# olsonanl/signature_kmers

Measured on AMD Instinct MI355X. Metric: k-mers/sec (extract+hash+count) at 1/2/4/8 GPUs; achieved HBM GB/s %, higher is better.
Workload: dtype u8

## Files before the change

### signature_kmers_amd/csrc/skm_build.hip

```cpp
#include <hip/hip_runtime.h>

#include <algorithm>
#include <type_traits>
#include <chrono>
#include <cmath>
#include <cstdio>
#include <cstdlib>
#include <cstring>
#include <deque>
#include <functional>
#include <memory>
#include <numeric>
#include <string>
#include <thread>
#include <vector>

#include "skm_common.h"
#include "skm_pool.h"
#include "skm_output.h"
#include "skm_util.h"

#if defined(SKM_WITH_RCCL)
#include <rccl/rccl.h>
#endif
// ... 2098 lines not shown
        }
#pragma unroll
        for (int t = 0; t < SC_POS; ++t)
            rk[t] = agg_rank(L.cnt, sb[t], base + threadIdx.x + (uint64_t)t * EX_THREADS < end);
        __syncthreads();
        const uint32_t tot = stage_reserve(L, nsub, cur1, b0 << sub_bits);
#pragma unroll
        for (int t = 0; t < SC_POS; ++t) {
            const uint64_t j = base + threadIdx.x + (uint64_t)t * EX_THREADS;
            if (j < end) {
                const uint32_t slot = L.off[sb[t]] + rk[t];
                L.hi[slot] = eh[t];
                L.lo[slot] = el[t];
                L.dst[slot] = (uint8_t)sb[t];
            }
        }
        __syncthreads();
        for (uint32_t j = threadIdx.x; j < tot; j += blockDim.x) {
            const uint32_t d = L.dst[j];
            const uint64_t o = L.base[d] + (j - L.off[d]);
            out_hi[o] = L.hi[j];
            out_lo[o] = L.lo[j];
        }
        __syncthreads();
    }
}

__global__ void k_colsum(const uint32_t* __restrict__ hist, uint32_t nwg, uint32_t NB, uint32_t* __restrict__ partial) {
    uint32_t b = blockIdx.x * blockDim.x + threadIdx.x;
    uint32_t rb = blockIdx.y;
    if (b >= NB) return;
    uint32_t w0 = rb * SCAN_ROWS, w1 = min(nwg, w0 + SCAN_ROWS);
    uint32_t s = 0;
    for (uint32_t w = w0; w < w1; ++w) s += hist[(uint64_t)w * NB + b];
    partial[(uint64_t)rb * NB + b] = s;
}

__global__ void k_bstart(const uint32_t* __restrict__ partial, uint32_t nrb, uint32_t NB, int b1_bits,
                         uint32_t* __restrict__ rbbase, uint32_t* __restrict__ bstart, uint64_t* __restrict__ owner_start,
                         uint32_t nowners) {
    __shared__ uint32_t s_wave[34];
    __shared__ unsigned long long s_tot[64];
    const uint32_t per = (NB + blockDim.x - 1) / blockDim.x;
    const uint32_t b0 = threadIdx.x * per;
    uint32_t local = 0;
    for (uint32_t b = b0; b < min(NB, b0 + per); ++b) {
        uint32_t acc = 0;
        for (uint32_t rb = 0; rb < nrb; ++rb) {
            uint32_t v = partial[(uint64_t)rb * NB + b];
            rbbase[(uint64_t)rb * NB + b] = acc;
            acc += v;
        }
        bstart[b] = acc;
        local += acc;
    }
    uint32_t total;
    uint32_t ex = wg_exclusive_scan(local, s_wave, total);
    uint32_t run = ex;
    for (uint32_t b = b0; b < min(NB, b0 + per); ++b) {
        uint32_t t = bstart[b];
        bstart[b] = run;
        run += t;
    }
    __syncthreads();
    if (threadIdx.x < nowners) {
        uint32_t ob = threadIdx.x << b1_bits;
        s_tot[threadIdx.x] = bstart[ob];
    }
    if (threadIdx.x == 0) s_tot[nowners] = total;
    __syncthreads();
    if (threadIdx.x <= nowners) owner_start[threadIdx.x] = s_tot[threadIdx.x];
    for (uint32_t b = b0; b < min(NB, b0 + per); ++b) {
        uint32_t o = b >> b1_bits;
        uint32_t rel = bstart[b] - (uint32_t)s_tot[o];
        for (uint32_t rb = 0; rb < nrb; ++rb) rbbase[(uint64_t)rb * NB + b] += rel;
    }
    __syncthreads();
    for (uint32_t b = b0; b < min(NB, b0 + per); ++b) bstart[b] -= (uint32_t)s_tot[b >> b1_bits];
    if (threadIdx.x == 0) bstart[NB] = 0;
}

__global__ void k_coloffs(const uint32_t* __restrict__ hist, const uint32_t* __restrict__ rbbase, uint32_t nwg, uint32_t NB,
                          uint32_t* __restrict__ offs) {
    uint32_t b = blockIdx.x * blockDim.x + threadIdx.x;
    uint32_t rb = blockIdx.y;
    if (b >= NB) return;
    uint32_t w0 = rb * SCAN_ROWS, w1 = min(nwg, w0 + SCAN_ROWS);
    uint32_t run = rbbase[(uint64_t)rb * NB + b];
    for (uint32_t w = w0; w < w1; ++w) {
        uint64_t idx = (uint64_t)w * NB + b;
        uint32_t v = hist[idx];
        offs[idx] = run;
        run += v;
    }
}

struct BucketArgs {
    uint64_t* recs_hi;
    const uint64_t* recs_lo;
    uint64_t* tmp_hi;
    uint64_t* tmp_lo;
    const uint64_t* bstart;
    const uint64_t* seg_start;
    const uint32_t* seg_len;
    uint32_t nsrc;
    uint32_t* sub_tab;
    unsigned long long* kept_ctr;

    uint32_t nbuckets;
    uint32_t bucket_base;
    int rem_bits;
    const uint32_t* glen;
    uint8_t* flags;
    unsigned long long* ctr;
    uint64_t* out_keys;
    skm_stored_kmer_data* out_data;
    Job* jobs;
    uint32_t* lens;
    OvfEntry* ovf;
    uint32_t ovf_cap;
    unsigned long long* stamps;
    uint64_t* big_desc;
    uint32_t big_cap;
    unsigned long long* big_ctr;
    int prio;
    int pshift;
    int flag_check;
    const uint32_t* skip;
    uint32_t sub_target;
    int diag;
    const uint32_t* order;
    int part_class;
};

#define SKM_STAMP(i)                                                          \
    do {                                                                      \
        if (A.stamps && threadIdx.x == 0) {                                   \
            const uint64_t _t = __builtin_amdgcn_s_memtime();                 \
            atomicAdd(&A.stamps[(i)], (unsigned long long)(_t - *L.tlast));   \
            *L.tlast = _t;                                                    \
        }                                                                     \
    } while (0)

constexpr uint32_t JOB_KEPT = 0x8000u;
constexpr uint32_t JOB_COUNT_MASK = 0x0FFFu;

struct SubLds {
    uint64_t* hi;
    uint64_t* lo;
    uint32_t* tab;
    uint16_t* slot;
    uint16_t* rank;
    uint16_t* goff;
    uint16_t* glist;
    uint16_t* order;
    uint16_t* big;
    uint32_t* wave;
    uint32_t* nbig;
    uint64_t* tlast;
    uint32_t* ccnt;
    uint32_t* lens32;
    uint64_t lens_sel;
};

__device__ __forceinline__ uint64_t kept_hi(uint64_t h43, uint32_t avg) { return (1ull << 63) | (h43 << 16) | avg; }
__device__ __forceinline__ uint64_t kept_lo(uint32_t f, uint32_t mean, uint32_t med, uint32_t var) {
    return (uint64_t)f | ((uint64_t)mean << 16) | ((uint64_t)med << 32) | ((uint64_t)var << 48);
}

__device__ __forceinline__ void write_kept(const BucketArgs& A, uint64_t o, uint64_t H, uint64_t L) {
    A.out_keys[o] = (H >> 16) & KEY_MASK;
    skm_stored_kmer_data d;
    d.avg_from_end = (uint16_t)(H & 0xFFFFu);
    d.function_index = (uint16_t)(L & 0xFFFFu);
    d.mean = (uint16_t)(L >> 16);
    d.median = (uint16_t)(L >> 32);
    d.var = (uint16_t)(L >> 48);
    A.out_data[o] = d;
}



__device__ __forceinline__ uint64_t shfl_xor_u64(uint64_t v, int m) {
    return ((uint64_t)(uint32_t)__shfl_xor((int)(uint32_t)(v >> 32), m, 64) << 32) |
           (uint32_t)__shfl_xor((int)(uint32_t)v, m, 64);
}


__device__ __forceinline__ void bm_combine(uint32_t& cand, uint32_t& cc) {
#pragma unroll
    for (int d = 1; d < 64; d <<= 1) {
        const uint32_t oc = xs(cand, d), on = xs(cc, d);
        if (oc == cand) {
            cc += on;
        } else if (cc >= on) {
            cc -= on;
        } else {
            cand = oc;
            cc = on - cc;
        }
    }
    cand = (uint32_t)__shfl((int)cand, 0, 64);
}


template <int S>
__device__ __forceinline__ uint64_t seg_bitonic64(uint64_t key, uint32_t& pay, uint32_t m) {
#pragma unroll
    for (int k = 2; k <= S; k <<= 1) {
#pragma unroll
        for (int j = k >> 1; j > 0; j >>= 1) {
            const uint64_t ok = xs64(key, j);
            const uint32_t op = xs(pay, j);
            const bool take_min = ((m & (uint32_t)j) == 0) == ((m & (uint32_t)k) == 0);
            if (take_min ? (ok < key) : (ok > key)) {
                key = ok;
                pay = op;
            }
        }
    }
    return key;
}

template <int S>
__device__ __forceinline__ uint32_t seg_bitonic32(uint32_t key, uint32_t m) {
#pragma unroll
    for (int k = 2; k <= S; k <<= 1) {
#pragma unroll
        for (int j = k >> 1; j > 0; j >>= 1) {
            const uint32_t ok = xs(key, j);
            const bool take_min = ((m & (uint32_t)j) == 0) == ((m & (uint32_t)k) == 0);
            key = take_min ? min(key, ok) : max(key, ok);
        }
    }
    return key;
}

template <int S>
__device__ __forceinline__ uint32_t seg_reduce_max(uint32_t x) {
#pragma unroll
    for (int d = 1; d < S; d <<= 1) x = max(x, xs(x, d));
    return x;
}

template <int S>
__device__ __forceinline__ uint32_t seg_reduce_sum(uint32_t x) {
#pragma unroll
    for (int d = 1; d < S; d <<= 1) x += xs(x, d);
    return x;
}

template <int S>
__device__ __forceinline__ void seg_groups(const SubLds& L, uint32_t q0, uint32_t qend, uint32_t G, uint32_t M,
                                           const BucketArgs& A, uint64_t hprefix, uint32_t* jobinfo,
                                           uint32_t* fmean) {
    const uint32_t lane = threadIdx.x & 63u;
    const uint32_t m = lane & (uint32_t)(S - 1);
    const uint32_t sbase = lane - m;
    const uint32_t q = q0 + lane / (uint32_t)S;
    const bool gv = q < qend;
    uint32_t rep = 0, a = 0, c = 0;
    if (gv) {
        const uint32_t g = L.big[q];
        rep = L.glist[g];
        a = L.goff[rep];
        c = (g + 1 < G ? L.goff[L.glist[g + 1]] : M) - a;
    }
    const bool real = gv && m < c;
    uint64_t key = ~0ull;
    uint32_t pay = 0;
    if (real) {
        const uint32_t j = L.order[a + m];
        const uint64_t hj = L.hi[j], lj = L.lo[j];
        key = ((hj & 0xFFFFull) << 48) | (lj >> 16);
        pay = (uint32_t)(hj >> 47);
    }
    key = seg_bitonic64<S>(key, pay, m);
    const uint32_t f = (uint32_t)(key >> 48);
    const uint32_t fprev = (uint32_t)__shfl_up((int)f, 1, 64);
    const bool head = !real || m == 0 || f != fprev;
    const uint64_t H = __ballot(head);
    const uint64_t above = lane == 63 ? 0ull : (H & ~((2ull << lane) - 1ull));
    const uint32_t nh = above ? (uint32_t)__ffsll((long long)above) - 1u : 64u;
    const uint32_t rlen = min(nh, sbase + c) - lane;
    const uint32_t v = (real && head) ? ((rlen << 16) | (0xFFFFu - f)) : 0u;
    const uint32_t best = seg_reduce_max<S>(v);
    const uint32_t cbest = best >> 16, bf = 0xFFFFu - (best & 0xFFFFu);
    const bool kept = gv && !((float)cbest < float(c) * 0.8f);
    const bool inrun = real && f == bf;
    const uint32_t len16 = pay >> 1;
    const uint32_t sum = seg_reduce_sum<S>(inrun ? len16 : 0u);
    const uint32_t i = (uint32_t)(key & ((1u << ELEM_I_BITS) - 1));
    const uint32_t off = real ? ((len16 - i) & 0xFFFFu) : 0x10000u;
    const uint32_t osort = seg_bitonic32<S>(off, m);
    const uint32_t avg = (uint32_t)__shfl((int)osort, (int)(sbase + (c >> 1)), 64);
    const uint64_t R = __ballot(inrun);
    const uint64_t segmask = (S == 64) ? ~0ull : (((1ull << S) - 1ull) << sbase);
    const uint64_t Rs = R & segmask;
    const uint32_t rs = Rs ? (uint32_t)__ffsll((long long)Rs) - 1u : sbase;
    const uint32_t s = (uint32_t)(key >> ELEM_I_BITS) & ((1u << ELEM_S_BITS) - 1u);
    const uint32_t fl = (A.flag_check && real && A.flags) ? A.flags[s] : 0u;
    const uint32_t len = (pay & 1u) ? A.glen[s] : len16;
    if (kept && real && fl == 0 && A.flags) mark_seq(A.flags, s);
    const uint32_t x0 = (uint32_t)__shfl((int)len, (int)(rs + cbest - 1), 64);
    const uint32_t x1 = (uint32_t)__shfl((int)len, (int)rs, 64);
    if (kept && inrun && cbest >= 3) L.lens32[2 * a + (rs + cbest - 1 - lane)] = len;
    if (kept && m == 0) {
        GRes r;
        r.kept = true;
        r.best_f = bf;
        r.cbest = cbest;
        r.avg = avg;
        r.mean = d2u16((double)(uint16_t)sum / (double)cbest);
        stats_small(r, x0, cbest == 2 ? x1 : 0u, cbest);
        const uint64_t h43 = key_h43(hprefix, (L.hi[rep] >> 16) & REM_MASK, A.rem_bits, A.pshift);
        L.hi[rep] = kept_hi(h43, r.avg);
        if (cbest >= 3) {
            jobinfo[rep] = (a << 16) | JOB_KEPT | cbest;
            fmean[rep] = bf | ((uint32_t)r.mean << 16);
        } else {
            jobinfo[rep] = JOB_KEPT;
            L.lo[rep] = kept_lo(bf, r.mean, r.median, r.var);
        }
    }
}

constexpr uint32_t LPER = CAP / BPK_THREADS;

__device__ __forceinline__ void load_batch(const uint64_t* __restrict__ src_hi, const uint64_t* __restrict__ src_lo,
                                           uint32_t n, uint64_t (&eh)[LPER], uint64_t (&el)[LPER]) {
#pragma unroll
    for (uint32_t u = 0; u < LPER; ++u) {
        const uint32_t j = threadIdx.x + u * BPK_THREADS;
        if (j < n) {
            eh[u] = __builtin_nontemporal_load(src_hi + j);
            el[u] = __builtin_nontemporal_load(src_lo + j);
        }
    }
}

__device__ __forceinline__ uint32_t process_sub(const uint64_t* __restrict__ src_hi, const uint64_t* __restrict__ src_lo,
                                            uint32_t n, const BucketArgs& A, uint64_t hprefix, const SubLds& L) {
    const uint32_t tid = threadIdx.x, nt = blockDim.x;
    const uint32_t EMPTY = 0xFFFFFFFFu;
    uint64_t eh[LPER], el[LPER];
    load_batch(src_hi, src_lo, n, eh, el);
    for (uint32_t t = tid; t < (uint32_t)TAB; t += nt) L.tab[t] = EMPTY;
#pragma unroll
    for (uint32_t u = 0; u < LPER; ++u) {
        const uint32_t j = tid + u * BPK_THREADS;
        if (j < n) {
            L.hi[j] = eh[u];
            L.lo[j] = el[u];
        }
    }
    if (tid == 0) *L.nbig = 0;
    if (tid < 8) L.ccnt[tid] = 0;
    __syncthreads();
    SKM_STAMP(2);
    for (uint32_t j = tid; j < n; j += nt) {
        const uint32_t rem = (uint32_t)(L.hi[j] >> 16) & REM_MASK;
        uint32_t slot = (rem * 0x9E3779B1u) >> (32 - TAB_BITS);
        uint32_t rk = 0;
        while (true) {
            const uint32_t cur = atomicCAS(&L.tab[slot], EMPTY, (j << 16) | 1u);
            if (cur == EMPTY) break;
            if (((uint32_t)(L.hi[cur >> 16] >> 16) & REM_MASK) == rem) {
                rk = atomicAdd(&L.tab[slot], 1u) & 0xFFFFu;
                break;
            }
            slot = (slot + 1) & (TAB - 1);
        }
        L.slot[j] = (uint16_t)slot;
        L.rank[j] = (uint16_t)rk;
    }
    __syncthreads();
    SKM_STAMP(3);
    uint32_t M = 0, G = 0;
    {
        const uint32_t j0 = tid * LPER;
        uint32_t ev[LPER], loc = 0;
#pragma unroll
        for (uint32_t u = 0; u < LPER; ++u) {
            const uint32_t j = j0 + u;
            ev[u] = j < n ? L.tab[L.slot[j]] : 0u;
            const uint32_t cnt = ev[u] & 0xFFFFu;
            loc += (cnt > 1 && (ev[u] >> 16) == j) ? ((cnt << 13) | 1u) : 0u;
        }
        uint32_t tot;
        uint32_t v = wg_exclusive_scan1(loc, L.wave, tot);
        uint32_t ms[LPER];
#pragma unroll
        for (uint32_t u = 0; u < LPER; ++u) {
            const uint32_t j = j0 + u;
            const uint32_t cnt = ev[u] & 0xFFFFu;
            ms[u] = 0xFFFFFFFFu;
            if (j < n && cnt > 1 && (ev[u] >> 16) == j) {
                L.goff[j] = (uint16_t)(v >> 13);
                L.glist[v & 0x1FFFu] = (uint16_t)j;
                v += (cnt << 13) | 1u;
            } else if (j < n && cnt == 1) {
                const uint64_t H = L.hi[j], Lo = L.lo[j];
                ms[u] = (uint32_t)(Lo >> 36);
                L.hi[j] = kept_hi(key_h43(hprefix, (H >> 16) & REM_MASK, A.rem_bits, A.pshift), (uint32_t)(Lo & 0xFFFFu));
                L.lo[j] = kept_lo((uint32_t)(H & 0xFFFFu), d2u16((double)(uint16_t)(H >> 48) / 1.0), 0, 0);
                L.rank[j] = 0xFFFFu;
            }
        }
        if (A.flags) mark_seqs<LPER>(A.flags, A.flag_check, ms);
        M = tot >> 13;
        G = tot & 0x1FFFu;
    }
    __syncthreads();
    SKM_STAMP(4);
    for (uint32_t j = tid; j < n; j += nt) {
        const uint32_t e = L.tab[L.slot[j]];
        if ((e & 0xFFFFu) > 1) L.order[L.goff[e >> 16] + L.rank[j]] = (uint16_t)j;
    }
    uint32_t* ccnt = L.ccnt;
    auto cls_of = [](uint32_t c) -> uint32_t {
        return c > 64u ? 6u : 31u - (uint32_t)__clz(c - 1u) - 0u;
    };
    for (uint32_t g = tid; g < G; g += nt) {
        const uint32_t a = L.goff[L.glist[g]];
        const uint32_t c = g + 1 < G ? L.goff[L.glist[g + 1]] - a : M - a;
        atomicAdd(&ccnt[cls_of(c)], 1u);
    }
    __syncthreads();
    SKM_STAMP(5);
    uint32_t* jobinfo = L.tab;
    uint32_t* fmean = L.tab + CAP;
    for (uint32_t j = tid; j < n; j += nt) jobinfo[j] = L.rank[j] == 0xFFFFu ? JOB_KEPT : 0u;
    uint32_t* cstart = ccnt + 8;
    uint32_t* tstart = ccnt + 16;
    if (tid == 0) {
        uint32_t run = 0, acc = 0;
        for (int q = 0; q < 7; ++q) {
            const uint32_t t = ccnt[q];
            ccnt[q] = run;
            cstart[q] = run;
            tstart[q] = acc;
            const uint32_t per = q < 6 ? (64u >> (q + 1)) : 1u;
            acc += (t + per - 1) / per;
            run += t;
        }
        cstart[7] = run;
        tstart[7] = acc;
    }
    unsigned long long big_base = 0;
    if (tid == 0 && cstart[7] > cstart[6]) big_base = atomicAdd(A.big_ctr, (unsigned long long)(cstart[7] - cstart[6]));
    __syncthreads();
    for (uint32_t g = tid; g < G; g += nt) {
        const uint32_t a = L.goff[L.glist[g]];
        const uint32_t c = g + 1 < G ? L.goff[L.glist[g + 1]] - a : M - a;
        L.big[atomicAdd(&ccnt[cls_of(c)], 1u)] = (uint16_t)g;
    }
    if (tid == 0) *reinterpret_cast<unsigned long long*>(L.wave + 44) = big_base;
    __syncthreads();
    SKM_STAMP(6);
    {
        const uint32_t ntask = tstart[6];
        const uint32_t nbig = cstart[7] - cstart[6];
        const uint64_t bbase = *reinterpret_cast<const unsigned long long*>(L.wave + 44);
        const uint32_t wave = tid >> 6, nwaves = nt >> 6, lane = tid & 63u;
        uint64_t* slots = reinterpret_cast<uint64_t*>(L.lens32);
        uint64_t* slots_lo = const_cast<uint64_t*>(src_lo);
        (void)wave;
        (void)nwaves;
        for (;;) {
            uint32_t t = 0;
            if (lane == 0) t = atomicAdd(&ccnt[7], 1u);
            t = (uint32_t)__builtin_amdgcn_readfirstlane((int)t);
            if (t >= nbig + ntask) break;
            if (t < nbig) {
                const uint32_t g = L.big[cstart[6] + t];
                const uint32_t rep = L.glist[g];
                const uint32_t a = L.goff[rep];
                const uint32_t c = g + 1 < G ? L.goff[L.glist[g + 1]] - a : M - a;
                for (uint32_t u = lane; u < c; u += 64) {
                    const uint32_t j = L.order[a + u];
                    const uint64_t hj = L.hi[j], lj = L.lo[j];
                    slots[a + u] = ((hj & 0xFFFFull) << 48) | (lj >> 16);
                    slots_lo[a + u] = elem_len(hj, lj, A.glen);
                }
                const uint64_t q = bbase + t;
                if (lane == 0 && q < A.big_cap) {
                    A.big_desc[2 * q] = key_h43(hprefix, (L.hi[rep] >> 16) & REM_MASK, A.rem_bits, A.pshift) |
                                        ((uint64_t)c << KEY_BITS);
                    A.big_desc[2 * q + 1] = L.lens_sel + 2 * a;
                }
                continue;
            }
            const uint32_t ts = ntask - 1u - (t - nbig);
            uint32_t k = 0;
            while (k < 5 && ts >= tstart[k + 1]) ++k;
            const uint32_t per = 64u >> (k + 1);
            const uint32_t q0 = cstart[k] + (ts - tstart[k]) * per, qe = cstart[k + 1];
            switch (k) {
                case 0: seg_groups<2>(L, q0, qe, G, M, A, hprefix, jobinfo, fmean); break;
                case 1: seg_groups<4>(L, q0, qe, G, M, A, hprefix, jobinfo, fmean); break;
                case 2: seg_groups<8>(L, q0, qe, G, M, A, hprefix, jobinfo, fmean); break;
                case 3: seg_groups<16>(L, q0, qe, G, M, A, hprefix, jobinfo, fmean); break;
                case 4: seg_groups<32>(L, q0, qe, G, M, A, hprefix, jobinfo, fmean); break;
                default: seg_groups<64>(L, q0, qe, G, M, A, hprefix, jobinfo, fmean); break;
            }
        }
    }
    __syncthreads();
    SKM_STAMP(11);
    SKM_STAMP(7);
    constexpr uint32_t EMIT_PER = CAP / BPK_THREADS;
    unsigned long long* s_base = reinterpret_cast<unsigned long long*>(L.wave + 36);
    const uint32_t j0 = tid * EMIT_PER;
    uint32_t cnt = 0;
#pragma unroll
    for (uint32_t u = 0; u < EMIT_PER; ++u) {
        const uint32_t j = j0 + u;
        const uint32_t jb = j < n ? jobinfo[j] : 0u;
        cnt += ((jb & JOB_KEPT) ? 1u : 0u) | ((jb & JOB_COUNT_MASK) ? 0x10000u : 0u);
    }
    uint32_t tot;
    const uint32_t pos = wg_exclusive_scan1(cnt, L.wave, tot);
    unsigned long long rsv = 0;
    if (tid == 0 && (tot & 0xFFFFu)) rsv = atomicAdd(A.kept_ctr, (unsigned long long)(tot & 0xFFFFu));
    if (tid == 64 && (tot >> 16)) rsv = atomicAdd(&A.ctr[3], (unsigned long long)(tot >> 16));
    {
        uint32_t pk = pos & 0xFFFFu, pj = pos >> 16;
#pragma unroll
        for (uint32_t u = 0; u < EMIT_PER; ++u) {
            const uint32_t jb = j0 + u < n ? jobinfo[j0 + u] : 0u;
            if (!(jb & JOB_KEPT)) continue;
            L.slot[pk] = (uint16_t)(j0 + u);
            if (jb & JOB_COUNT_MASK) {
                L.order[pj++] = (uint16_t)(j0 + u);
                L.rank[j0 + u] = (uint16_t)pk;
            }
            ++pk;
        }
    }
    if (tid == 0 || tid == 64) s_base[tid >> 6] = rsv;
    __syncthreads();
    const uint32_t nkept = tot & 0xFFFFu, njob = tot >> 16;
    if (nkept) {
        const uint64_t ob = s_base[0];
#pragma unroll 1
        for (uint32_t t = tid; t < nkept; t += nt) {
            const uint32_t j = L.slot[t];
            const uint32_t jb = jobinfo[j];
            uint64_t lo;
            if (jb & JOB_COUNT_MASK) {
                const uint32_t fm = fmean[j];
                lo = kept_lo(fm & 0xFFFFu, fm >> 16, 0, 0);
            } else {
                lo = L.lo[j];
            }
            write_kept(A, ob + t, L.hi[j], lo);
        }
        const uint64_t jbase = njob ? s_base[1] : 0;
#pragma unroll 1
        for (uint32_t t = tid; t < njob; t += nt) {
            const uint32_t j = L.order[t];
            const uint32_t jb = jobinfo[j];
            Job jbr;
            jbr.lens_off = L.lens_sel + 2 * (jb >> 16);
            jbr.n = jb & JOB_COUNT_MASK;
            jbr.out_idx = (uint32_t)(ob + L.rank[j]);
            A.jobs[jbase + t] = jbr;
        }
    }
    __syncthreads();
    SKM_STAMP(8);
    return nkept;
}

struct SubMem {
    uint64_t hi[CAP];
    uint64_t lo[CAP];
    uint32_t tab[TAB];
    __align__(16) uint16_t slot[CAP];
    __align__(16) uint16_t rank[CAP];
    __align__(16) uint16_t goff[CAP];
    __align__(16) uint16_t glist[CAP];
    __align__(16) uint16_t order[CAP];
    __align__(16) uint16_t big[CAP / 2];
    __align__(16) uint32_t wave[48];
    uint32_t nbig;
    uint64_t tlast;
    uint32_t ccnt[24];
};

__device__ __forceinline__ SubLds sub_lds(SubMem& m) {
    SubLds L;
    L.ccnt = m.ccnt;
    L.tlast = &m.tlast;
    if (threadIdx.x == 0) m.tlast = __builtin_amdgcn_s_memtime();
    L.hi = m.hi;
    L.lo = m.lo;
    L.tab = m.tab;
    L.slot = m.slot;
    L.rank = m.rank;
    L.goff = m.goff;
    L.glist = m.glist;
    L.order = m.order;
    L.big = m.big;
    L.wave = m.wave;
    L.nbig = &m.nbig;
    L.lens32 = nullptr;
    L.lens_sel = 0;
    return L;
}

__global__ __launch_bounds__(BPK_THREADS, BPK_WAVES_EU) void k_bucket_process(BucketArgs A) {
    static_assert(CAP % BPK_THREADS == 0, "emit assigns CAP / BPK_THREADS elements per thread");
    __shared__ SubMem s_mem;
    __shared__ uint32_t s_sub[(1 << MAX_B2) + 1];
    if (A.skip && *A.skip) return;
    SubLds L = sub_lds(s_mem);

    const uint32_t bucket = blockIdx.x;
    if (bucket >= A.nbuckets) return;
    const uint64_t r0 = A.bstart[bucket], r1 = A.bstart[bucket + 1];
    const uint64_t n = r1 - r0;
    if (n == 0) return;
    const uint64_t hprefix = (uint64_t)(A.bucket_base + bucket) << A.rem_bits;
    if (A.prio == 1) __builtin_amdgcn_s_setprio(1);
    if (A.prio == 2) __builtin_amdgcn_s_setprio(2);
    if (A.prio >= 3) __builtin_amdgcn_s_setprio(3);

    const bool direct = n <= (uint64_t)CAP && A.nsrc == 1;
    uint32_t nsub = 1;
    if (!direct) {
        const uint32_t* tab = A.sub_tab + (uint64_t)bucket * SUB_TAB;
        nsub = tab[0];
        for (uint32_t d = threadIdx.x; d <= nsub; d += blockDim.x) s_sub[d] = tab[1 + d];
        __syncthreads();
        SKM_STAMP(9);
    }
    struct Batch {
        uint32_t a, cnt;
    };
    auto next_batch = [&](uint32_t& d) -> Batch {
        if (direct) {
            if (d >= 1) return Batch{0, 0};
            d = 1;
            return Batch{0, (uint32_t)n};
        }
        while (d < nsub) {
            const uint32_t a = s_sub[d];
            if (s_sub[d + 1] - a == 0 || s_sub[d + 1] - a > (uint32_t)CAP) {
                ++d;
                continue;
            }
            uint32_t d2 = d + 1;
            while (d2 < nsub && s_sub[d2 + 1] - a <= (uint32_t)CAP) ++d2;
            d = d2;
            return Batch{a, s_sub[d2] - a};
        }
        return Batch{0, 0};
    };
    const uint64_t* base_hi = direct ? A.recs_hi + r0 : A.tmp_hi + r0;
    const uint64_t* base_lo = direct ? A.recs_lo + r0 : A.tmp_lo + r0;
    const uint64_t sel = direct ? LENS_IN_RECS : LENS_IN_TMP;
    uint32_t d = 0;
    for (Batch cur = next_batch(d); cur.cnt; cur = next_batch(d)) {
        L.lens_sel = (sel << LENS_SEL_SHIFT) | (2 * (r0 + cur.a));
        L.lens32 = reinterpret_cast<uint32_t*>(const_cast<uint64_t*>(base_hi + cur.a));
        process_sub(base_hi + cur.a, base_lo + cur.a, cur.cnt, A, hprefix, L);
        __syncthreads();
        SKM_STAMP(10);
    }
}

struct BigOut {
    uint64_t h43;
    uint64_t lens_off;
    uint32_t n;
    uint16_t avg, func, mean, pad0;
    uint32_t pad1;
};
static_assert(sizeof(BigOut) == 32, "BigOut layout");

struct BigArgs {
    const uint64_t* desc;
    const unsigned long long* ndesc;
    uint32_t cap;
    const uint64_t* recs_hi;
    const uint64_t* tmp_hi;
    const uint64_t* recs_lo;
    const uint64_t* tmp_lo;
    uint8_t* flags;
    BigOut* out;
};

template <int E>
__device__ __forceinline__ uint32_t ballot_count(const bool (&p)[E]) {
    uint32_t n = 0;
#pragma unroll
    for (int e = 0; e < E; ++e) n += (uint32_t)__popcll(__ballot(p[e]));
    return n;
}

template <int E, int D>
__device__ __forceinline__ void bitonic_cross(uint64_t (&ky)[E], bool take_min) {
#pragma unroll
    for (int e = 0; e < E; ++e) {
        const uint64_t o = xshfl64<D>(ky[e]);
        ky[e] = take_min ? (o < ky[e] ? o : ky[e]) : (o > ky[e] ? o : ky[e]);
    }
}

template <int E>
__device__ __forceinline__ void big_group(const BigArgs& B, uint64_t g, uint64_t* mem, const uint64_t* mlen,
                                          uint32_t c, uint64_t h43, uint64_t lens_off) {
    const uint32_t lane = threadIdx.x & 63u;
    uint32_t fo[E];
    uint64_t ky[E];
#pragma unroll
    for (int e = 0; e < E; ++e) {
        const uint32_t t = lane * E + (uint32_t)e;
        fo[e] = 0xFFFFFFFFu;
        ky[e] = ~0ull;
        if (t < c) {
            const uint64_t v = mem[t];
            const uint32_t len = (uint32_t)mlen[t];
            const uint32_t i = (uint32_t)v & ((1u << ELEM_I_BITS) - 1u);
            fo[e] = ((uint32_t)(v >> 48) << 16) | ((len - i) & 0xFFFFu);
            ky[e] = (v << 16) | t;
        }
    }
    uint32_t cand = 0xFFFFFFFFu, cc = 0;
#pragma unroll
    for (int e = 0; e < E; ++e) {
        if (fo[e] != 0xFFFFFFFFu) {
            const uint32_t f = fo[e] >> 16;
            if (cc == 0) {
                cand = f;
                cc = 1;
            } else if (f == cand) {
                ++cc;
            } else {
                --cc;
            }
        }
    }
    bm_combine(cand, cc);
    bool p[E];
#pragma unroll
    for (int e = 0; e < E; ++e) p[e] = (fo[e] >> 16) == cand;
    const uint32_t nb = ballot_count<E>(p);
    BigOut o;
    o.h43 = h43;
    o.lens_off = lens_off;
    o.n = 0;
    o.avg = o.func = o.mean = 0;
    o.pad0 = 0;
    o.pad1 = 0;
    if ((float)nb < float(c) * 0.8f) {
// ... 4492 lines not shown
```

Baseline: 11.70 billion.

## Process two segmented-sort tasks per wave with runtime segment sizes

Replaces the per-size templated segmented bitonic sort/reduce with a runtime-sized version that handles two group tasks per wavefront at once. Compares are turned into ballot masks, and asm pins keep the two independent shuffle chains interleaved to hide cross-lane latency. Groups are now described by packed (offset,count) words built during the scan, with class counts taken there too, which drops the glist/big arrays and a separate counting pass. qdesc reuses the goff storage, and the extra masking and uniform-value handling add per-step ALU work.

Result: no change. 11.67 billion (-0.2%).

```diff
diff --git a/signature_kmers_amd/csrc/skm_build.hip b/signature_kmers_amd/csrc/skm_build.hip
--- a/signature_kmers_amd/csrc/skm_build.hip
+++ b/signature_kmers_amd/csrc/skm_build.hip
@@ -2274,9 +2274,9 @@
     uint16_t* slot;
     uint16_t* rank;
     uint16_t* goff;
-    uint16_t* glist;
+    uint32_t* gdesc;
+    uint32_t* qdesc;
     uint16_t* order;
-    uint16_t* big;
     uint32_t* wave;
     uint32_t* nbig;
     uint64_t* tlast;
@@ -2326,123 +2326,220 @@
 }
 
 
-template <int S>
-__device__ __forceinline__ uint64_t seg_bitonic64(uint64_t key, uint32_t& pay, uint32_t m) {
-#pragma unroll
-    for (int k = 2; k <= S; k <<= 1) {
+struct SegTask {
+    uint32_t ls;
+    uint32_t q0;
+    uint32_t qe;
+};
+
+constexpr uint64_t lanes_with(int b) {
+    uint64_t m = 0;
+    for (int l = 0; l < 64; ++l)
+        if (l & b) m |= 1ull << l;
+    return m;
+}
+
+#ifndef SKM_SEG_PIN
+#define SKM_SEG_PIN 1
+#endif
+template <class T>
+__device__ __forceinline__ void stage_pin(T& a, T& b) {
+#if SKM_SEG_PIN
+    asm volatile("" : "+v"(a), "+v"(b));
+#else
+    __builtin_amdgcn_sched_barrier(0);
+#endif
+}
+__device__ __forceinline__ void stage_pin(uint64_t& a, uint64_t& b, uint32_t& c, uint32_t& d) {
+#if SKM_SEG_PIN
+    asm volatile("" : "+v"(a), "+v"(b), "+v"(c), "+v"(d));
+#else
+    __builtin_amdgcn_sched_barrier(0);
+#endif
+}
+
+__device__ __forceinline__ bool lane_of(uint64_t uniform_mask) {
+    return __builtin_amdgcn_inverse_ballot_w64(uniform_mask);
+}
+
+__device__ __forceinline__ void seg_bitonic64x2(uint64_t (&key)[2], uint32_t (&pay)[2], const uint32_t (&S)[2],
+                                                uint32_t smax) {
+#pragma unroll
+    for (int k = 2; k <= 64; k <<= 1) {
+        if ((uint32_t)k > smax) break;
+        uint64_t on[2], desc[2];
+#pragma unroll
+        for (int t = 0; t < 2; ++t) {
+            on[t] = (uint32_t)k <= S[t] ? ~0ull : 0ull;
+            desc[t] = (uint32_t)k < S[t] ? lanes_with(k) : 0ull;
+        }
 #pragma unroll
         for (int j = k >> 1; j > 0; j >>= 1) {
-            const uint64_t ok = xs64(key, j);
-            const uint32_t op = xs(pay, j);
-            const bool take_min = ((m & (uint32_t)j) == 0) == ((m & (uint32_t)k) == 0);
-            if (take_min ? (ok < key) : (ok > key)) {
-                key = ok;
-                pay = op;
-            }
-        }
-    }
-    return key;
-}
-
-template <int S>
-__device__ __forceinline__ uint32_t seg_bitonic32(uint32_t key, uint32_t m) {
-#pragma unroll
-    for (int k = 2; k <= S; k <<= 1) {
+            uint64_t ok[2];
+            uint32_t op[2];
+#pragma unroll
+            for (int t = 0; t < 2; ++t) {
+                ok[t] = xs64(key[t], j);
+                op[t] = xs(pay[t], j);
+            }
+            stage_pin(ok[0], ok[1], op[0], op[1]);
+#pragma unroll
+            for (int t = 0; t < 2; ++t) {
+                const bool take = lane_of((__ballot(ok[t] < key[t]) ^ lanes_with(j) ^ desc[t]) & on[t]);
+                key[t] = take ? ok[t] : key[t];
+                pay[t] = take ? op[t] : pay[t];
+            }
+            stage_pin(key[0], key[1], pay[0], pay[1]);
+        }
+    }
+}
+
+__device__ __forceinline__ void seg_bitonic32x2(uint32_t (&key)[2], const uint32_t (&S)[2], uint32_t smax) {
+#pragma unroll
+    for (int k = 2; k <= 64; k <<= 1) {
+        if ((uint32_t)k > smax) break;
+        uint64_t on[2], desc[2];
+#pragma unroll
+        for (int t = 0; t < 2; ++t) {
+            on[t] = (uint32_t)k <= S[t] ? ~0ull : 0ull;
+            desc[t] = (uint32_t)k < S[t] ? lanes_with(k) : 0ull;
+        }
 #pragma unroll
         for (int j = k >> 1; j > 0; j >>= 1) {
-            const uint32_t ok = xs(key, j);
-            const bool take_min = ((m & (uint32_t)j) == 0) == ((m & (uint32_t)k) == 0);
-            key = take_min ? min(key, ok) : max(key, ok);
-        }
-    }
-    return key;
-}
-
-template <int S>
-__device__ __forceinline__ uint32_t seg_reduce_max(uint32_t x) {
-#pragma unroll
-    for (int d = 1; d < S; d <<= 1) x = max(x, xs(x, d));
-    return x;
-}
-
-template <int S>
-__device__ __forceinline__ uint32_t seg_reduce_sum(uint32_t x) {
-#pragma unroll
-    for (int d = 1; d < S; d <<= 1) x += xs(x, d);
-    return x;
-}
-
-template <int S>
-__device__ __forceinline__ void seg_groups(const SubLds& L, uint32_t q0, uint32_t qend, uint32_t G, uint32_t M,
-                                           const BucketArgs& A, uint64_t hprefix, uint32_t* jobinfo,
-                                           uint32_t* fmean) {
+            uint32_t ok[2];
+#pragma unroll
+            for (int t = 0; t < 2; ++t) ok[t] = xs(key[t], j);
+            stage_pin(ok[0], ok[1]);
+#pragma unroll
+            for (int t = 0; t < 2; ++t) {
+                const bool take = lane_of((__ballot(ok[t] < key[t]) ^ lanes_with(j) ^ desc[t]) & on[t]);
+                key[t] = take ? ok[t] : key[t];
+            }
+            stage_pin(key[0], key[1]);
+        }
+    }
+}
+
+__device__ __forceinline__ void seg_reduce_max2(uint32_t (&x)[2], const uint32_t (&S)[2], uint32_t smax) {
+#pragma unroll
+    for (int d = 1; d < 64; d <<= 1) {
+        if ((uint32_t)d >= smax) break;
+        uint32_t o[2];
+#pragma unroll
+        for (int t = 0; t < 2; ++t) o[t] = xs(x[t], d);
+        stage_pin(o[0], o[1]);
+#pragma unroll
+        for (int t = 0; t < 2; ++t) x[t] = max(x[t], (uint32_t)d < S[t] ? o[t] : 0u);
+    }
+}
+
+__device__ __forceinline__ void seg_reduce_sum2(uint32_t (&x)[2], const uint32_t (&S)[2], uint32_t smax) {
+#pragma unroll
+    for (int d = 1; d < 64; d <<= 1) {
+        if ((uint32_t)d >= smax) break;
+        uint32_t o[2];
+#pragma unroll
+        for (int t = 0; t < 2; ++t) o[t] = xs(x[t], d);
+        stage_pin(o[0], o[1]);
+#pragma unroll
+        for (int t = 0; t < 2; ++t) x[t] += (uint32_t)d < S[t] ? o[t] : 0u;
+    }
+}
+
+__device__ __forceinline__ void seg_groups2(const SubLds& L, const SegTask (&T)[2], const BucketArgs& A,
+                                            uint64_t hprefix, uint32_t* jobinfo, uint32_t* fmean) {
     const uint32_t lane = threadIdx.x & 63u;
-    const uint32_t m = lane & (uint32_t)(S - 1);
-    const uint32_t sbase = lane - m;
-    const uint32_t q = q0 + lane / (uint32_t)S;
-    const bool gv = q < qend;
-    uint32_t rep = 0, a = 0, c = 0;
-    if (gv) {
-        const uint32_t g = L.big[q];
-        rep = L.glist[g];
-        a = L.goff[rep];
-        c = (g + 1 < G ? L.goff[L.glist[g + 1]] : M) - a;
-    }
-    const bool real = gv && m < c;
-    uint64_t key = ~0ull;
-    uint32_t pay = 0;
-    if (real) {
-        const uint32_t j = L.order[a + m];
+    uint32_t S[2], m[2], sbase[2], a[2], c[2], rep[2], pay[2], jm[2];
+    uint64_t key[2];
+    bool gv[2], real[2];
+    const uint32_t smax = 1u << max(T[0].ls, T[1].ls);
+#pragma unroll
+    for (int t = 0; t < 2; ++t) {
+        S[t] = T[t].ls ? 1u << T[t].ls : 0u;
+        m[t] = lane & (S[t] - 1u);
+        sbase[t] = lane - m[t];
+        const uint32_t q = T[t].q0 + (lane >> T[t].ls);
+        gv[t] = q < T[t].qe;
+        const uint32_t d = L.qdesc[gv[t] ? q : 0u];
+        a[t] = gv[t] ? (d & 0xFFFFu) : 0u;
+        c[t] = gv[t] ? (d >> 16) : 0u;
+        real[t] = m[t] < c[t];
+    }
+#pragma unroll
+    for (int t = 0; t < 2; ++t) jm[t] = L.order[real[t] ? a[t] + m[t] : 0u];
+#pragma unroll
+    for (int t = 0; t < 2; ++t) {
+        const uint32_t j = real[t] ? jm[t] : 0u;
+        rep[t] = j;
         const uint64_t hj = L.hi[j], lj = L.lo[j];
-        key = ((hj & 0xFFFFull) << 48) | (lj >> 16);
-        pay = (uint32_t)(hj >> 47);
-    }
-    key = seg_bitonic64<S>(key, pay, m);
-    const uint32_t f = (uint32_t)(key >> 48);
-    const uint32_t fprev = (uint32_t)__shfl_up((int)f, 1, 64);
-    const bool head = !real || m == 0 || f != fprev;
-    const uint64_t H = __ballot(head);
-    const uint64_t above = lane == 63 ? 0ull : (H & ~((2ull << lane) - 1ull));
-    const uint32_t nh = above ? (uint32_t)__ffsll((long long)above) - 1u : 64u;
-    const uint32_t rlen = min(nh, sbase + c) - lane;
-    const uint32_t v = (real && head) ? ((rlen << 16) | (0xFFFFu - f)) : 0u;
-    const uint32_t best = seg_reduce_max<S>(v);
-    const uint32_t cbest = best >> 16, bf = 0xFFFFu - (best & 0xFFFFu);
-    const bool kept = gv && !((float)cbest < float(c) * 0.8f);
-    const bool inrun = real && f == bf;
-    const uint32_t len16 = pay >> 1;
-    const uint32_t sum = seg_reduce_sum<S>(inrun ? len16 : 0u);
-    const uint32_t i = (uint32_t)(key & ((1u << ELEM_I_BITS) - 1));
-    const uint32_t off = real ? ((len16 - i) & 0xFFFFu) : 0x10000u;
-    const uint32_t osort = seg_bitonic32<S>(off, m);
-    const uint32_t avg = (uint32_t)__shfl((int)osort, (int)(sbase + (c >> 1)), 64);
-    const uint64_t R = __ballot(inrun);
-    const uint64_t segmask = (S == 64) ? ~0ull : (((1ull << S) - 1ull) << sbase);
-    const uint64_t Rs = R & segmask;
-    const uint32_t rs = Rs ? (uint32_t)__ffsll((long long)Rs) - 1u : sbase;
-    const uint32_t s = (uint32_t)(key >> ELEM_I_BITS) & ((1u << ELEM_S_BITS) - 1u);
-    const uint32_t fl = (A.flag_check && real && A.flags) ? A.flags[s] : 0u;
-    const uint32_t len = (pay & 1u) ? A.glen[s] : len16;
-    if (kept && real && fl == 0 && A.flags) mark_seq(A.flags, s);
-    const uint32_t x0 = (uint32_t)__shfl((int)len, (int)(rs + cbest - 1), 64);
-    const uint32_t x1 = (uint32_t)__shfl((int)len, (int)rs, 64);
-    if (kept && inrun && cbest >= 3) L.lens32[2 * a + (rs + cbest - 1 - lane)] = len;
-    if (kept && m == 0) {
-        GRes r;
-        r.kept = true;
-        r.best_f = bf;
-        r.cbest = cbest;
-        r.avg = avg;
-        r.mean = d2u16((double)(uint16_t)sum / (double)cbest);
-        stats_small(r, x0, cbest == 2 ? x1 : 0u, cbest);
-        const uint64_t h43 = key_h43(hprefix, (L.hi[rep] >> 16) & REM_MASK, A.rem_bits, A.pshift);
-        L.hi[rep] = kept_hi(h43, r.avg);
-        if (cbest >= 3) {
-            jobinfo[rep] = (a << 16) | JOB_KEPT | cbest;
-            fmean[rep] = bf | ((uint32_t)r.mean << 16);
-        } else {
-            jobinfo[rep] = JOB_KEPT;
-            L.lo[rep] = kept_lo(bf, r.mean, r.median, r.var);
+        key[t] = real[t] ? (((hj & 0xFFFFull) << 48) | (lj >> 16)) : ~0ull;
+        pay[t] = real[t] ? (uint32_t)(hj >> 47) : 0u;
+    }
+    seg_bitonic64x2(key, pay, S, smax);
+    uint32_t f[2], v[2];
+#pragma unroll
+    for (int t = 0; t < 2; ++t) {
+        f[t] = (uint32_t)(key[t] >> 48);
+        const uint32_t fprev = (uint32_t)__shfl_up((int)f[t], 1, 64);
+        const bool head = !real[t] || m[t] == 0 || f[t] != fprev;
+        const uint64_t H = __ballot(head);
+        const uint64_t above = lane == 63 ? 0ull : (H & ~((2ull << lane) - 1ull));
+        const uint32_t nh = above ? (uint32_t)__ffsll((long long)above) - 1u : 64u;
+        const uint32_t rlen = min(nh, sbase[t] + c[t]) - lane;
+        v[t] = (real[t] && head) ? ((rlen << 16) | (0xFFFFu - f[t])) : 0u;
+    }
+    seg_reduce_max2(v, S, smax);
+    uint32_t cbest[2], bf[2], len16[2], sum[2], off[2];
+    bool kept[2], inrun[2];
+#pragma unroll
+    for (int t = 0; t < 2; ++t) {
+        cbest[t] = v[t] >> 16;
+        bf[t] = 0xFFFFu - (v[t] & 0xFFFFu);
+        kept[t] = gv[t] && !((float)cbest[t] < float(c[t]) * 0.8f);
+        inrun[t] = real[t] && f[t] == bf[t];
+        len16[t] = pay[t] >> 1;
+        sum[t] = inrun[t] ? len16[t] : 0u;
+        const uint32_t i = (uint32_t)(key[t] & ((1u << ELEM_I_BITS) - 1));
+        off[t] = real[t] ? ((len16[t] - i) & 0xFFFFu) : 0x10000u;
+    }
+    seg_reduce_sum2(sum, S, smax);
+    seg_bitonic32x2(off, S, smax);
+    uint32_t avg[2], rs[2], s[2], fl[2], len[2];
+#pragma unroll
+    for (int t = 0; t < 2; ++t) {
+        avg[t] = (uint32_t)__shfl((int)off[t], (int)(sbase[t] + (c[t] >> 1)), 64);
+        const uint64_t R = __ballot(inrun[t]);
+        const uint64_t segmask = S[t] == 64u ? ~0ull : (((1ull << S[t]) - 1ull) << sbase[t]);
+        const uint64_t Rs = R & segmask;
+        rs[t] = Rs ? (uint32_t)__ffsll((long long)Rs) - 1u : sbase[t];
+        s[t] = (uint32_t)(key[t] >> ELEM_I_BITS) & ((1u << ELEM_S_BITS) - 1u);
+        fl[t] = (A.flag_check && real[t] && A.flags) ? A.flags[s[t]] : 0u;
+        len[t] = (pay[t] & 1u) ? A.glen[s[t]] : len16[t];
+    }
+#pragma unroll
+    for (int t = 0; t < 2; ++t) {
+        if (kept[t] && real[t] && fl[t] == 0 && A.flags) mark_seq(A.flags, s[t]);
+        const uint32_t x0 = (uint32_t)__shfl((int)len[t], (int)(rs[t] + cbest[t] - 1), 64);
+        const uint32_t x1 = (uint32_t)__shfl((int)len[t], (int)rs[t], 64);
+        if (kept[t] && inrun[t] && cbest[t] >= 3)
+            L.lens32[2 * a[t] + (rs[t] + cbest[t] - 1 - lane)] = len[t];
+        if (kept[t] && m[t] == 0) {
+            GRes r;
+            r.kept = true;
+            r.best_f = bf[t];
+            r.cbest = cbest[t];
+            r.avg = avg[t];
+            r.mean = d2u16((double)(uint16_t)sum[t] / (double)cbest[t]);
+            stats_small(r, x0, cbest[t] == 2 ? x1 : 0u, cbest[t]);
+            const uint64_t h43 = key_h43(hprefix, (L.hi[rep[t]] >> 16) & REM_MASK, A.rem_bits, A.pshift);
+            L.hi[rep[t]] = kept_hi(h43, r.avg);
+            if (cbest[t] >= 3) {
+                jobinfo[rep[t]] = (a[t] << 16) | JOB_KEPT | cbest[t];
+                fmean[rep[t]] = bf[t] | ((uint32_t)r.mean << 16);
+            } else {
+                jobinfo[rep[t]] = JOB_KEPT;
+                L.lo[rep[t]] = kept_lo(bf[t], r.mean, r.median, r.var);
+            }
         }
     }
 }
@@ -2498,7 +2595,11 @@
     }
     __syncthreads();
     SKM_STAMP(3);
-    uint32_t M = 0, G = 0;
+    uint32_t* ccnt = L.ccnt;
+    auto cls_of = [](uint32_t c) -> uint32_t {
+        return c > 64u ? 6u : 31u - (uint32_t)__clz(c - 1u);
+    };
+    uint32_t G = 0;
     {
         const uint32_t j0 = tid * LPER;
         uint32_t ev[LPER], loc = 0;
@@ -2519,44 +2620,27 @@
             ms[u] = 0xFFFFFFFFu;
             if (j < n && cnt > 1 && (ev[u] >> 16) == j) {
                 L.goff[j] = (uint16_t)(v >> 13);
-                L.glist[v & 0x1FFFu] = (uint16_t)j;
+                L.gdesc[v & 0x1FFFu] = (v >> 13) | (cnt << 16);
+                atomicAdd(&ccnt[cls_of(cnt)], 1u);
                 v += (cnt << 13) | 1u;
             } else if (j < n && cnt == 1) {
                 const uint64_t H = L.hi[j], Lo = L.lo[j];
                 ms[u] = (uint32_t)(Lo >> 36);
                 L.hi[j] = kept_hi(key_h43(hprefix, (H >> 16) & REM_MASK, A.rem_bits, A.pshift), (uint32_t)(Lo & 0xFFFFu));
-                L.lo[j] = kept_lo((uint32_t)(H & 0xFFFFu), d2u16((double)(uint16_t)(H >> 48) / 1.0), 0, 0);
+                L.lo[j] = kept_lo((uint32_t)(H & 0xFFFFu), (uint32_t)(uint16_t)(H >> 48), 0, 0);
                 L.rank[j] = 0xFFFFu;
             }
         }
         if (A.flags) mark_seqs<LPER>(A.flags, A.flag_check, ms);
-        M = tot >> 13;
         G = tot & 0x1FFFu;
     }
     __syncthreads();
     SKM_STAMP(4);
-    for (uint32_t j = tid; j < n; j += nt) {
-        const uint32_t e = L.tab[L.slot[j]];
-        if ((e & 0xFFFFu) > 1) L.order[L.goff[e >> 16] + L.rank[j]] = (uint16_t)j;
-    }
-    uint32_t* ccnt = L.ccnt;
-    auto cls_of = [](uint32_t c) -> uint32_t {
-        return c > 64u ? 6u : 31u - (uint32_t)__clz(c - 1u) - 0u;
-    };
-    for (uint32_t g = tid; g < G; g += nt) {
-        const uint32_t a = L.goff[L.glist[g]];
-        const uint32_t c = g + 1 < G ? L.goff[L.glist[g + 1]] - a : M - a;
-        atomicAdd(&ccnt[cls_of(c)], 1u);
-    }
-    __syncthreads();
-    SKM_STAMP(5);
-    uint32_t* jobinfo = L.tab;
-    uint32_t* fmean = L.tab + CAP;
-    for (uint32_t j = tid; j < n; j += nt) jobinfo[j] = L.rank[j] == 0xFFFFu ? JOB_KEPT : 0u;
     uint32_t* cstart = ccnt + 8;
     uint32_t* tstart = ccnt + 16;
+    unsigned long long big_base = 0;
     if (tid == 0) {
-        uint32_t run = 0, acc = 0;
+        uint32_t run = 0, acc = 0, nb = 0;
         for (int q = 0; q < 7; ++q) {
             const uint32_t t = ccnt[q];
             ccnt[q] = run;
@@ -2565,40 +2649,49 @@
             const uint32_t per = q < 6 ? (64u >> (q + 1)) : 1u;
             acc += (t + per - 1) / per;
             run += t;
+            nb = t;
         }
         cstart[7] = run;
         tstart[7] = acc;
-    }
-    unsigned long long big_base = 0;
-    if (tid == 0 && cstart[7] > cstart[6]) big_base = atomicAdd(A.big_ctr, (unsigned long long)(cstart[7] - cstart[6]));
+        if (nb) big_base = atomicAdd(A.big_ctr, (unsigned long long)nb);
+    }
+    for (uint32_t j = tid; j < n; j += nt) {
+        const uint32_t e = L.tab[L.slot[j]];
+        if ((e & 0xFFFFu) > 1) L.order[L.goff[e >> 16] + L.rank[j]] = (uint16_t)j;
+    }
     __syncthreads();
+    SKM_STAMP(5);
+    uint32_t* jobinfo = L.tab;
+    uint32_t* fmean = L.tab + CAP;
+    for (uint32_t j = tid; j < n; j += nt) jobinfo[j] = L.rank[j] == 0xFFFFu ? JOB_KEPT : 0u;
     for (uint32_t g = tid; g < G; g += nt) {
-        const uint32_t a = L.goff[L.glist[g]];
-        const uint32_t c = g + 1 < G ? L.goff[L.glist[g + 1]] - a : M - a;
-        L.big[atomicAdd(&ccnt[cls_of(c)], 1u)] = (uint16_t)g;
+        const uint32_t d = L.gdesc[g];
+        L.qdesc[atomicAdd(&ccnt[cls_of(d >> 16)], 1u)] = d;
     }
     if (tid == 0) *reinterpret_cast<unsigned long long*>(L.wave + 44) = big_base;
     __syncthreads();
     SKM_STAMP(6);
     {
-        const uint32_t ntask = tstart[6];
-        const uint32_t nbig = cstart[7] - cstart[6];
+        auto uni = [](uint32_t x) -> uint32_t { return (uint32_t)__builtin_amdgcn_readfirstlane((int)x); };
+        const uint32_t ntask = uni(tstart[6]);
+        const uint32_t nbig = uni(cstart[7] - cstart[6]);
         const uint64_t bbase = *reinterpret_cast<const unsigned long long*>(L.wave + 44);
-        const uint32_t wave = tid >> 6, nwaves = nt >> 6, lane = tid & 63u;
+        const uint32_t lane = tid & 63u;
         uint64_t* slots = reinterpret_cast<uint64_t*>(L.lens32);
         uint64_t* slots_lo = const_cast<uint64_t*>(src_lo);
-        (void)wave;
-        (void)nwaves;
+        uint32_t ts_of[5];
+#pragma unroll
+        for (int k = 0; k < 5; ++k) ts_of[k] = uni(tstart[k + 1]);
+        const uint32_t ntick = nbig + (ntask + 1u) / 2u;
         for (;;) {
             uint32_t t = 0;
             if (lane == 0) t = atomicAdd(&ccnt[7], 1u);
-            t = (uint32_t)__builtin_amdgcn_readfirstlane((int)t);
-            if (t >= nbig + ntask) break;
+            t = uni(t);
+            if (t >= ntick) break;
             if (t < nbig) {
-                const uint32_t g = L.big[cstart[6] + t];
-                const uint32_t rep = L.glist[g];
-                const uint32_t a = L.goff[rep];
-                const uint32_t c = g + 1 < G ? L.goff[L.glist[g + 1]] - a : M - a;
+                const uint32_t d = L.qdesc[cstart[6] + t];
+                const uint32_t a = d & 0xFFFFu, c = d >> 16;
+                const uint32_t rep = L.order[a];
                 for (uint32_t u = lane; u < c; u += 64) {
                     const uint32_t j = L.order[a + u];
                     const uint64_t hj = L.hi[j], lj = L.lo[j];
@@ -2613,19 +2706,26 @@
                 }
                 continue;
             }
-            const uint32_t ts = ntask - 1u - (t - nbig);
-            uint32_t k = 0;
-            while (k < 5 && ts >= tstart[k + 1]) ++k;
-            const uint32_t per = 64u >> (k + 1);
-            const uint32_t q0 = cstart[k] + (ts - tstart[k]) * per, qe = cstart[k + 1];
-            switch (k) {
-                case 0: seg_groups<2>(L, q0, qe, G, M, A, hprefix, jobinfo, fmean); break;
-                case 1: seg_groups<4>(L, q0, qe, G, M, A, hprefix, jobinfo, fmean); break;
-                case 2: seg_groups<8>(L, q0, qe, G, M, A, hprefix, jobinfo, fmean); break;
-                case 3: seg_groups<16>(L, q0, qe, G, M, A, hprefix, jobinfo, fmean); break;
-                case 4: seg_groups<32>(L, q0, qe, G, M, A, hprefix, jobinfo, fmean); break;
-                default: seg_groups<64>(L, q0, qe, G, M, A, hprefix, jobinfo, fmean); break;
-            }
+            SegTask T[2];
+            uint32_t k[2], ts[2];
+#pragma unroll
+            for (int s = 0; s < 2; ++s) {
+                const uint32_t x = 2u * (t - nbig) + (uint32_t)s;
+                ts[s] = ntask - 1u - min(x, ntask - 1u);
+                k[s] = 0;
+#pragma unroll
+                for (int i = 0; i < 5; ++i) k[s] += ts[s] >= ts_of[i] ? 1u : 0u;
+            }
+#pragma unroll
+            for (int s = 0; s < 2; ++s) {
+                const bool on = 2u * (t - nbig) + (uint32_t)s < ntask;
+                const uint32_t q0 = uni(cstart[k[s]] + ((ts[s] - tstart[k[s]]) << (5u - k[s])));
+                const uint32_t qe = uni(cstart[k[s] + 1]);
+                T[s].ls = on ? k[s] + 1u : 0u;
+                T[s].q0 = on ? q0 : 0u;
+                T[s].qe = on ? qe : 0u;
+            }
+            seg_groups2(L, T, A, hprefix, jobinfo, fmean);
         }
     }
     __syncthreads();
@@ -2702,9 +2802,8 @@
     __align__(16) uint16_t slot[CAP];
     __align__(16) uint16_t rank[CAP];
     __align__(16) uint16_t goff[CAP];
-    __align__(16) uint16_t glist[CAP];
+    __align__(16) uint32_t gdesc[CAP / 2];
     __align__(16) uint16_t order[CAP];
-    __align__(16) uint16_t big[CAP / 2];
     __align__(16) uint32_t wave[48];
     uint32_t nbig;
     uint64_t tlast;
@@ -2722,9 +2821,9 @@
     L.slot = m.slot;
     L.rank = m.rank;
     L.goff = m.goff;
-    L.glist = m.glist;
+    L.gdesc = m.gdesc;
+    L.qdesc = reinterpret_cast<uint32_t*>(m.goff);
     L.order = m.order;
-    L.big = m.big;
     L.wave = m.wave;
     L.nbig = &m.nbig;
     L.lens32 = nullptr;
```
